# WL-Amigo/waifu2x-converter-cpp

Measured on AMD Instinct MI355X. Metric: Mpixels/sec end-to-end scale2.0x 7-layer conv, higher is better.
Workload: dtype f32; 1 GPU; scale2x_1080p (BASELINE.json configs[1]): scale2.0x topology (1-32-32-64-64-128-128-1, synthetic seeded weights) on a 1920x1080 RGB frame -> Y plane nearest-2x -> 3840x2160 CNN plane, one frame per GPU per step

## Files before the change

waifu2x-converter-cpp_amd/csrc/w2xc_wino4_body.inc:

```
    static_assert(!PROG || FUSE7, "PROG finishes the fused last layer");
    constexpr int ROWS = 16;
    constexpr int NST = CIN / 4;
    constexpr int NOB = COUT / 64;
    constexpr int CHS = 168;
    constexpr int RAW_PIECES = 11;
    constexpr unsigned RAW_BYTES = RAW_PIECES * 1024;
    constexpr unsigned U_BASE = 3 * RAW_BYTES, U_BYTES = 36 * 1024;
    constexpr unsigned V_BASE = U_BASE + 2 * U_BYTES, V_BYTES = 18 * 1024;
    constexpr unsigned SPARE_BASE = V_BASE + 2 * V_BYTES;
    constexpr unsigned BIAS_BASE = SPARE_BASE + V_BYTES;
    static_assert(CIN % 16 == 0 && COUT % 64 == 0 && NST % 4 == 0 && NST >= 8, "planes");
    constexpr int STRIP = 16;
    constexpr int GW = 8;
    constexpr unsigned TRIG_BASE = BIAS_BASE + COUT * 4;
    const int tiles_y = W4B_SEL(bd.items, nitems) / (NOB * tiles_x);
    W4B_ONLY(const int img_tiles = bd.items / NOB;)
    const int pxcd = blockIdx.x & 7;
    auto band_lo = [&](int k, int r) { return (k * tiles_x + (r & 7)) >> 3; };
    auto tile_coords = [&](int pt_, int &ty_, int &tx_) {
        W4B_ONLY(pt_ = pt_ % img_tiles;)
        if constexpr (PROG) {
            const int p8 = pt_ / tiles_x;
            int rem = pt_ - p8 * tiles_x, j = 0, lo = band_lo(pxcd, 0), wd = band_lo(pxcd + 1, 0) - lo;
            while (rem >= wd && j < 7) {
                rem -= wd;
                j++;
                lo = band_lo(pxcd, j);
                wd = band_lo(pxcd + 1, j) - lo;
            }
            ty_ = 8 * p8 + j;
            tx_ = lo + rem;
            return;
        }
        const int per_strip = STRIP * tiles_y;
        int sidx = pt_ / per_strip;
        const int nfull = tiles_x / STRIP;
        if (sidx > nfull) sidx = nfull;
        const int wid = sidx < nfull ? STRIP : tiles_x - nfull * STRIP;
        const int q = pt_ - sidx * per_strip;
        ty_ = q / wid;
        tx_ = sidx * STRIP + (q - ty_ * wid);
    };
    extern __shared__ __attribute__((aligned(16))) float lds[];
    const unsigned lds0 = (unsigned)(size_t)(__attribute__((address_space(3))) float *)lds;
    char *ldsb = reinterpret_cast<char *>(lds);

    const int lane = threadIdx.x & 63;
    const int wave = __builtin_amdgcn_readfirstlane(threadIdx.x >> 6);
    const int pt = wave & 3, bt = wave >> 2;
    const unsigned b_voff = (unsigned)lane * 16u;
    auto lin = [&]() { unsigned v = b_voff; asm volatile("" : "+v"(v)); return v; };
    auto lane_o = [&]() { return (int)(lin() >> 4); };

    const int xcd = blockIdx.x & 7, per = gridDim.x >> 3;
    const int cq = nitems >> 3, cr = nitems & 7;
    int chunk_begin = xcd < cr ? xcd * (cq + 1) : cr * (cq + 1) + (xcd - cr) * cq;
    int chunk_end = chunk_begin + cq + (xcd < cr ? 1 : 0);
    if constexpr (PROG) {
        int nloc = (tiles_y >> 3) * tiles_x;
        for (int j = 0; j < (tiles_y & 7); j++) nloc += band_lo(xcd + 1, j) - band_lo(xcd, j);
        chunk_begin = 0;
        chunk_end = nloc * NOB;
    }
#ifndef W4_PAIR
#define W4_PAIR 0
#endif
    int item0 = chunk_begin + (blockIdx.x >> 3);
    int nmy = (chunk_end - item0 + per - 1) / per;
    if constexpr (W4_PAIR && NOB == 2 && !PROG) {
        const int ntile = nitems >> 1, tq = ntile >> 3, tr = ntile & 7;
        const int tb = xcd < tr ? xcd * (tq + 1) : tr * (tq + 1) + (xcd - tr) * tq, te = tb + tq + (xcd < tr ? 1 : 0);
        item0 = tb + (blockIdx.x >> 3);
        if (item0 >= te) return;
        nmy = 2 * ((te - item0 + per - 1) / per);
    } else if (item0 >= chunk_end) return;
    auto item_of = [&](int n) {
        const int nn = n < nmy ? n : nmy - 1;
        if constexpr (W4_PAIR && NOB == 2 && !PROG) return 2 * (item0 + (nn >> 1) * per) + (nn & 1);
        else return item0 + nn * per;
    };

    for (int c = threadIdx.x; c < COUT; c += 512) lds[BIAS_BASE / 4 + c] = d.bias[c];
    if constexpr (PROG) {
        if (threadIdx.x < 4) lds[TRIG_BASE / 4 + threadIdx.x] = 0.0f;
    }

    const long long cs4 = d.in_cs * 4, rs4 = d.in_rs * 4;
    constexpr int DW = W4_DMA4 ? 4 : 8;
    constexpr int RJ = (RAW_PIECES + DW - 1) / DW;
    constexpr int UQ = 36 / DW + (36 % DW ? 1 : 0);
    unsigned voff[RJ];
    const char *a_base;
    int xlim_r;
    auto tile_offsets = [&](int it) {
        int ty_, tx_;
        tile_coords(it / NOB, ty_, tx_);
        const int lane_t = lane_o();
        const int y0 = ty_ * ROWS - d.wino_py + d.off_y, x0 = tx_ * 32 + d.off_x;
        const int yb = clampi(y0, 0, d.in_h - 1);
        a_base = reinterpret_cast<const char *>(d.in) + (long long)yb * rs4;
        W4B_ONLY(a_base += (long long)(it / bd.items) * bd.in_bs * 4;)
        xlim_r = d.in_w - x0;
        if constexpr (IN_NHWC) {
            xlim_r = 64;
#pragma unroll
            for (int jj = 0; jj < RJ; jj++) {
                int ci = (jj * DW + wave) * 64 + lane_t;
                ci = ci < (ROWS + 2) * 36 ? ci : (ROWS + 2) * 36 - 1;
                const int R = ci / 36, slot = ci - R * 36;
                const int x = 4 * (slot % 9) + slot / 9;
                const int gy = clampi(y0 + R, 0, d.in_h - 1) - yb;
                const int gx = clampi(x0 + x, 0, d.in_w - 1);
                voff[jj] = (unsigned)((long long)gy * rs4 + (long long)gx * (CIN * 4));
            }
            return;
        }
        const int xq_last = (d.in_w - 1) & ~3;
#pragma unroll
        for (int jj = 0; jj < RJ; jj++) {
            const int ci = (jj * DW + wave) * 64 + lane_t;
            int kk = ci / CHS;
            kk = kk < 4 ? kk : 3;
            const int rem = ci - kk * CHS;
            int R = rem / 9;
            const int q = rem - R * 9;
            R = R < ROWS + 2 ? R : ROWS + 1;
            const int gy = clampi(y0 + R, 0, d.in_h - 1) - yb;
            int gx = x0 + 4 * q;
            gx = gx < xq_last ? gx : xq_last;
            voff[jj] = (unsigned)((long long)kk * cs4 + (long long)gy * rs4 + (long long)gx * 4);
        }
    };
    const unsigned wbase = (unsigned)__builtin_amdgcn_readfirstlane(lds0 + (unsigned)wave * 1024u);
    auto dma_raw = [&](auto JJ, unsigned roff, int slice) {
        constexpr int jj = decltype(JJ)::value;
        const char *sbase = a_base + (long long)slice * (IN_NHWC ? 16 : 4 * cs4);
        lds_dma16_si<jj * DW * 1024u>(sbase, voff[jj], wbase + roff);
    };
    const char *wpk_w = reinterpret_cast<const char *>(d.wpk) + (size_t)wave * 1024;
    auto dma_u = [&](int ob, int s_, auto SLOT, auto Q) {
        constexpr unsigned slot = decltype(SLOT)::value;
        constexpr int q = decltype(Q)::value;
        const char *sbase = wpk_w + ((size_t)(ob * NST + s_) * 36 + q * DW) * 1024;
        lds_dma16_si<U_BASE + slot * U_BYTES + q * DW * 1024u>(sbase, b_voff, wbase);
    };
#ifndef W4_DMA_BASES
#define W4_DMA_BASES 1
#endif
    constexpr bool DMAB = W4_DMA_BASES && W4_DMA4 && !(CIN == 32 && COUT == 128 && !OUT_PLANAR && !IN_NHWC && !FUSE7);
    auto dma_u_pair = [&](const char *u_pair, auto SLOT, auto Q) {
        constexpr unsigned slot = decltype(SLOT)::value;
        constexpr int q = decltype(Q)::value;
        lds_dma16_sio<U_BASE + slot * U_BYTES + q * DW * 1024u, (q & 1) ? 0 : -(DW * 1024)>(u_pair, b_voff, wbase);
    };

    const unsigned ua_u = U_BASE + (unsigned)pt * 1024u, va_u = V_BASE + (unsigned)bt * 1024u;
#ifndef W4_KEEP_BASES
#define W4_KEEP_BASES 1
#endif
    unsigned ua0_v = b_voff + ua_u, ua1_v = b_voff + ua_u + U_BYTES, va_v = b_voff + va_u;
    asm volatile("" : "+v"(ua0_v), "+v"(ua1_v), "+v"(va_v));
    auto ua_of = [&](unsigned slot) { return W4_KEEP_BASES ? ldsb + (slot ? ua1_v : ua0_v) : ldsb + (lin() + (ua_u + slot * U_BYTES)); };
    auto va_of = [&](unsigned slot) { return W4_KEEP_BASES ? ldsb + va_v + slot * V_BYTES : ldsb + (lin() + (va_u + slot * V_BYTES)); };
#ifndef W4_KEEP_TR
#define W4_KEEP_TR 1
#endif
    auto tr_rd_calc = [&]() {
        const int l = lane_o(), tr_r = l >> 5, tr_k = (l >> 3) & 3, tr_c = l & 7;
        return IN_NHWC ? (unsigned)((4 * (2 * bt + tr_r) * 36 + tr_c) * 16 + tr_k * 4)
                       : (unsigned)((tr_k * CHS + 4 * (2 * bt + tr_r) * 9 + tr_c) * 16);
    };
    auto tr_wr_calc = [&]() {
        const int l = lane_o(), tr_r = l >> 5, tr_k = (l >> 3) & 3, tr_c = l & 7;
        return V_BASE + (unsigned)bt * 1024u + (unsigned)((tr_k * 16 + tr_r * 8 + tr_c) * 16);
    };
    unsigned tr_rd_v = tr_rd_calc(), tr_wr_v = tr_wr_calc();
    asm volatile("" : "+v"(tr_rd_v), "+v"(tr_wr_v));
    auto tr_rd = [&]() { return W4_KEEP_TR ? tr_rd_v : tr_rd_calc(); };
    auto tr_wr = [&]() { return W4_KEEP_TR ? tr_wr_v : tr_wr_calc(); };

    const int ngroups = (tiles_x + GW - 1) / GW;
    auto job_of_lane = [&](int item, int l, int &jr, int &jg) {
        int r, tx;
        tile_coords(item / NOB, r, tx);
        jr = r - (l & 1);
        jg = tx / GW - (l >> 1);
        return l < 4 && jr >= 0 && ((l >> 1) == 0 || ((tx & (GW - 1)) == 0 && tx > 0));
    };
    auto job_target = [&](int jr, int jg) {
        const int rows = jr + 1 < tiles_y ? 2 : 1;
        const int c1 = (jg + 1) * GW + 1;
        return NOB * rows * ((c1 < tiles_x ? c1 : tiles_x) - jg * GW);
    };
    const int njobs = tiles_y * ngroups;
    unsigned *const q_slots = d.prog_cnt + njobs, *const q_head = d.prog_cnt + 2 * njobs, *const q_tail = q_head + 1;
    unsigned *const lds_action = reinterpret_cast<unsigned *>(ldsb + TRIG_BASE), *const lds_ticket = lds_action + 1;
    constexpr int CW = 7;
    auto prog_early = [&](int item, unsigned &tick, unsigned &q0, unsigned &q1) {
        tick = 0xFFFFFFFFu;
        if (item >= 0) {
            int jr, jg;
            if (job_of_lane(item, lane_o(), jr, jg)) tick = __hip_atomic_fetch_add(d.prog_cnt + (jr * ngroups + jg), 1u, __ATOMIC_RELAXED, __HIP_MEMORY_SCOPE_AGENT);
        }
        const unsigned t = *lds_ticket;
        q0 = __hip_atomic_load(t ? q_slots + (t - 1) : q_head, __ATOMIC_RELAXED, __HIP_MEMORY_SCOPE_AGENT);
        q1 = __hip_atomic_load(q_tail, __ATOMIC_RELAXED, __HIP_MEMORY_SCOPE_AGENT);
    };
    auto prog_late = [&](int item, unsigned tick, unsigned q0, unsigned q1) {
        if (item >= 0) {
            int jr, jg;
            const bool valid = job_of_lane(item, lane_o(), jr, jg);
            if (valid && tick == (unsigned)(job_target(jr, jg) - 1)) {
                const unsigned slot = __hip_atomic_fetch_add(q_tail, 1u, __ATOMIC_RELAXED, __HIP_MEMORY_SCOPE_AGENT);
                __hip_atomic_store(q_slots + slot, (unsigned)(jr * ngroups + jg) + 1u, __ATOMIC_RELAXED, __HIP_MEMORY_SCOPE_AGENT);
            }
        }
        unsigned t = *lds_ticket, action = 0;
        if (t) {
            if (q0) { action = q0; t = 0; }
        } else if ((int)(q1 - q0) > 0) {
            unsigned h = 0;
            if (lane_o() == 0) h = __hip_atomic_fetch_add(q_head, 1u, __ATOMIC_RELAXED, __HIP_MEMORY_SCOPE_AGENT);
            h = (unsigned)__builtin_amdgcn_readfirstlane((int)h);
            t = h < (unsigned)njobs ? h + 1 : 0;
        }
        if (lane_o() == 0) { *lds_action = action; *lds_ticket = t; }
    };
    auto prog_run = [&]() {
        const unsigned action = (unsigned)__builtin_amdgcn_readfirstlane((int)*lds_action);
        if (action) {
            W4ProgJob a;
            a.G = d.out; a.ts = d.out_ts; a.gs = d.out_gs; a.rs = d.out_rs;
            a.out = d.g_out; a.out_rs = d.g_out_rs; a.bias = d.g_bias; a.flags = d.prog_flags; a.epoch = d.prog_epoch;
            a.g_h = d.g_h; a.g_w = d.g_w; a.g_off = d.g_off; a.wino_py = d.wino_py; a.ngroups = ngroups;
            w4_prog_job<NOB>(a, (int)(action - 1) / ngroups, (int)(action - 1) % ngroups);
        }
        return action;
    };

    float dd[36];
    auto raw_read = [&](const char *src, auto I_) {
        constexpr int i = decltype(I_)::value;
        if constexpr ((W4_ABL & 2) != 0) {
            static_for<0, 6>([&](auto JJ) { dd[i * 6 + decltype(JJ)::value] = (float)(i + decltype(JJ)::value); });
        } else if constexpr (IN_NHWC) {
            static_for<0, 6>([&](auto JJ) {
                constexpr int j = decltype(JJ)::value;
                dd[i * 6 + j] = *reinterpret_cast<const float *>(src + (i * 36 + (j & 3) * 9 + (j >> 2)) * 16);
            });
        } else {
            const f32x4 a = *reinterpret_cast<const f32x4 *>(src + i * 144);
            const f32x2 b = *reinterpret_cast<const f32x2 *>(src + i * 144 + 16);
            dd[i * 6 + 0] = a[0]; dd[i * 6 + 1] = a[1]; dd[i * 6 + 2] = a[2]; dd[i * 6 + 3] = a[3];
            dd[i * 6 + 4] = b[0]; dd[i * 6 + 5] = b[1];
        }
    };
    auto raw_mask = [&](int xlim) {
        if (xlim < 34) {
            const int lim = xlim - 4 * (lane_o() & 7);
            static_for<0, 36>([&](auto E) {
                constexpr int e = decltype(E)::value;
                dd[e] = (e % 6) < lim ? dd[e] : 0.0f;
            });
        }
    };
    auto row_pass = [&](auto I_) {
        constexpr int i = decltype(I_)::value;
        if constexpr (!(W4_ABL & 3)) bt6(dd[i * 6 + 0], dd[i * 6 + 1], dd[i * 6 + 2], dd[i * 6 + 3], dd[i * 6 + 4], dd[i * 6 + 5]);
        if constexpr (!(W4_ABL & 3)) asm volatile("" : "+v"(dd[i * 6 + 0]), "+v"(dd[i * 6 + 1]), "+v"(dd[i * 6 + 2]), "+v"(dd[i * 6 + 3]), "+v"(dd[i * 6 + 4]), "+v"(dd[i * 6 + 5]));
    };
    auto col_pass = [&](auto J_) {
        constexpr int j = decltype(J_)::value;
        if constexpr (!(W4_ABL & 3)) bt6(dd[0 * 6 + j], dd[1 * 6 + j], dd[2 * 6 + j], dd[3 * 6 + j], dd[4 * 6 + j], dd[5 * 6 + j]);
        if constexpr (!(W4_ABL & 3)) asm volatile("" : "+v"(dd[0 * 6 + j]), "+v"(dd[1 * 6 + j]), "+v"(dd[2 * 6 + j]), "+v"(dd[3 * 6 + j]), "+v"(dd[4 * 6 + j]), "+v"(dd[5 * 6 + j]));
    };
    auto v_write = [&](char *dst, auto Q_) {
        constexpr int q = decltype(Q_)::value;
        if constexpr (!(W4_ABL & 2))
        {
#ifdef W4_VW32
            static_for<0, 4>([&](auto E_) { constexpr int e = decltype(E_)::value; *reinterpret_cast<float *>(dst + q * 2048 + e * 4) = dd[w4p_dd_of(4 * q + e)]; });
#else
            *reinterpret_cast<f32x4 *>(dst + q * 2048) = f32x4{dd[w4p_dd_of(4 * q)], dd[w4p_dd_of(4 * q + 1)], dd[w4p_dd_of(4 * q + 2)], dd[w4p_dd_of(4 * q + 3)]};
#endif
        }
    };

    auto run = [&](auto PH_) {
    constexpr int PH = decltype(PH_)::value;
    using C0 = std::integral_constant<int, 0>;
    using C1 = std::integral_constant<int, 1>;
    using U0 = std::integral_constant<unsigned, 0u>;
    const unsigned park_u = (bt * 3 + PH - 1) < 4 ? U_BASE + U_BYTES + (unsigned)(bt * 3 + PH - 1) * 9216u : SPARE_BASE + (unsigned)(bt * 3 + PH - 1 - 4) * 9216u;
    auto park = [&]() {
        char *pa = ldsb + (lin() + park_u);
        static_for<0, 9>([&](auto Q_) {
            constexpr int q = decltype(Q_)::value;
            *reinterpret_cast<f32x4 *>(pa + q * 1024) = f32x4{dd[4 * q], dd[4 * q + 1], dd[4 * q + 2], dd[4 * q + 3]};
        });
    };
    auto unpark = [&]() {
        const char *pa = ldsb + (lin() + park_u);
        static_for<0, 9>([&](auto Q_) {
            constexpr int q = decltype(Q_)::value;
            const f32x4 v = *reinterpret_cast<const f32x4 *>(pa + q * 1024);
            dd[4 * q] = v[0]; dd[4 * q + 1] = v[1]; dd[4 * q + 2] = v[2]; dd[4 * q + 3] = v[3];
        });
    };
    auto quarter = [&](auto Q_, const char *src, char *dst, int xlim) {
        constexpr int q = decltype(Q_)::value;
        if constexpr (q == 0) {
            static_for<0, 6>([&](auto I) { raw_read(src, I); });
            raw_mask(xlim);
        }
        if constexpr (q < 2) static_for<3 * q, 3 * q + 3>([&](auto I) { row_pass(I); });
        else static_for<3 * (q - 2), 3 * (q - 2) + 3>([&](auto J) { col_pass(J); });
        if constexpr (q == 3) static_for<0, 9>([&](auto Q) { v_write(dst, Q); });
    };
    tile_offsets(item_of(0));
    int xlim_cur = xlim_r;
    auto raw_all = [&](unsigned roff, int slice) {
        if (wave < DW) {
            static_for<0, RJ - 1>([&](auto JJ) { dma_raw(JJ, roff, slice); });
            if (wave < RAW_PIECES - (RJ - 1) * DW) dma_raw(std::integral_constant<int, RJ - 1>{}, roff, slice);
        }
    };
    for (int sl = 0; sl < 3; sl++) raw_all((unsigned)sl * RAW_BYTES, sl);
    if (wave < DW) {
        const int ob0 = item_of(0) % NOB;
        static_for<0, UQ - 1>([&](auto Q) { dma_u(ob0, 0, U0{}, Q); });
        if (wave < 36 - (UQ - 1) * DW) dma_u(ob0, 0, U0{}, std::integral_constant<int, UQ - 1>{});
    }
    W2XC_WAIT_VMCNT(0);
    __builtin_amdgcn_s_barrier();
    asm volatile("" ::: "memory");
    if constexpr (PH < 3) {
        const char *src = ldsb + PH * RAW_BYTES + tr_rd();
        static_for<0, 4 - PH>([&](auto Q) { quarter(Q, src, ldsb + tr_wr(), xlim_cur); });
    }
    asm volatile("s_waitcnt lgkmcnt(0)" ::: "memory");
    __builtin_amdgcn_s_barrier();
    asm volatile("" ::: "memory");
    for (int sl = 3; sl < 6; sl++) raw_all((unsigned)(sl - 3) * RAW_BYTES, sl);
    W2XC_WAIT_VMCNT(0);
    __builtin_amdgcn_s_barrier();
    asm volatile("" ::: "memory");
    if constexpr (PH == 3) quarter(C0{}, ldsb + tr_rd(), nullptr, xlim_cur);
    asm volatile("s_waitcnt lgkmcnt(0)" ::: "memory");
    __builtin_amdgcn_s_barrier();
    asm volatile("" ::: "memory");

    constexpr int PF = W4_PF;
    static_assert(PF == 1 || PF == 2, "operand look-ahead");
    f32x4 a4[PF + 1], b4[PF + 1];
    auto load_first = [&](unsigned slot) {
        const char *ua = ua_of(slot);
        const char *va = va_of(slot);
        static_for<0, PF>([&](auto G) {
            constexpr int g = decltype(G)::value;
            const int b = PF == 2 ? g : (int)slot;
            a4[b] = *reinterpret_cast<const f32x4 *>(ua + g * 4096);
            b4[b] = *reinterpret_cast<const f32x4 *>(va + g * 2048);
        });
    };
    unsigned rd = RAW_BYTES, mid = 2 * RAW_BYTES, fr = 0;
    int stamp = 0;
    (void)stamp;
    W4_STAMP(stamp++);
    for (int n = 0; n < nmy; n++) {
        const int item = item_of(n), item_n = item_of(n + 1);
        f32x4 acc[36];

        auto stage = [&](auto J_, auto FIRST_, int s) {
            constexpr int J = decltype(J_)::value;
            constexpr bool FIRST = decltype(FIRST_)::value;
            constexpr int QT = (J - PH) & 3;
            constexpr unsigned par = J & 1, nxt = par ^ 1u;
            int u_ob = item % NOB, u_s = s + 1;
            if (s == NST - 1) { u_ob = item_n % NOB; u_s = 0; }
            const char *ua = ua_of(par);
            const char *va = va_of(par);
            const char *u_st = wpk_w + (size_t)(u_ob * NST + u_s) * 36864, *u_pair = u_st;
            if constexpr (DMAB) asm volatile("" : "+s"(u_st));
            const char *srcQ = nullptr;
            char *dstQ = nullptr;
            if constexpr (QT == 0) srcQ = ldsb + (rd + tr_rd());
            if constexpr (QT == 3) dstQ = ldsb + (tr_wr() + nxt * V_BYTES);
            const int xlimQ = s + 4 < NST ? xlim_cur : xlim_r;
            if constexpr (J == 2) {
                if (s == NST - 6) tile_offsets(item_n);
            }
            const int r_slice = s + 6 < NST ? s + 6 : s + 6 - NST;
            static_for<0, 36>([&](auto XI) {
                constexpr int xi = decltype(XI)::value;
                constexpr int g = xi >> 2;
                if constexpr (xi == 32) {
                    W4_STAMP(stamp++);
                    if constexpr ((W4_ABL & 32) != 0) W2XC_WAIT_VMCNT(0);
                    else if (wave < RAW_PIECES - (RJ - 1) * DW) wait_vmcnt_n(RJ);
                    else if (wave < DW) wait_vmcnt_n(RJ - 1);
                    asm volatile("s_waitcnt lgkmcnt(0)" ::: "memory");
                    W4_STAMP(stamp++);
                    __builtin_amdgcn_s_barrier();
                    asm volatile("" ::: "memory");
                    { const unsigned tr = rd; rd = mid; mid = fr; fr = tr; }
                    if (s != NST - 1) {
                        if constexpr (PF == 2) load_first(nxt);
                        else {
                            a4[nxt] = *reinterpret_cast<const f32x4 *>(ua_of(nxt));
                            b4[nxt] = *reinterpret_cast<const f32x4 *>(va_of(nxt));
                        }
                    }
                    W4_STAMP(stamp++);
                    __builtin_amdgcn_sched_barrier(0);
                }
                if constexpr ((xi & 3) == 0 && g + PF < 9 && !(W4_ABL & 128)) {
                    constexpr int b = PF == 2 ? (g + PF) % 3 : ((g + 1 + (int)par) & 1);
                    a4[b] = *reinterpret_cast<const f32x4 *>(ua + (g + PF) * 4096);
                    b4[b] = *reinterpret_cast<const f32x4 *>(va + (g + PF) * 2048);
                    __builtin_amdgcn_sched_barrier(0);
                }
                {
                    constexpr int b = PF == 2 ? g % 3 : ((g + (int)par) & 1);
                    if constexpr (FIRST) asm volatile("v_mfma_f32_16x16x4_f32 %0, %1, %2, 0" : "=v"(acc[xi]) : "v"(a4[b][xi & 3]), "v"(b4[b][xi & 3]));
                    else asm volatile("v_mfma_f32_16x16x4_f32 %0, %1, %2, %0" : "+v"(acc[xi]) : "v"(a4[b][xi & 3]), "v"(b4[b][xi & 3]));
                }
                __builtin_amdgcn_sched_barrier(0);
                constexpr int TSTEP = W4_DMA4 ? 1 : 2, tk = xi >= 1 && (xi - 1) % TSTEP == 0 ? (xi - 1) / TSTEP : -1;
                if constexpr (tk >= 0 && tk < UQ && !(W4_ABL & 16)) {
                    constexpr int q = tk;
                    if constexpr (DMAB) {
                        if (wave < (q == UQ - 1 ? 36 - (UQ - 1) * DW : DW)) {
                            if constexpr ((q & 1) == 0) {
                                u_pair = u_st + (q + 1) * (DW * 1024);
                                asm volatile("" : "+s"(u_pair));
                            }
                            dma_u_pair(u_pair, std::integral_constant<unsigned, nxt>{}, std::integral_constant<int, q>{});
                        }
                    } else {
                        if (wave < (q == UQ - 1 ? 36 - (UQ - 1) * DW : DW)) dma_u(u_ob, u_s, std::integral_constant<unsigned, nxt>{}, std::integral_constant<int, q>{});
                    }
                    __builtin_amdgcn_sched_barrier(0);
                }
                if constexpr (tk >= UQ && tk < UQ + RJ && !(W4_ABL & 32)) {
                    constexpr int jj = tk - UQ;
                    if (wave < (jj == RJ - 1 ? RAW_PIECES - (RJ - 1) * DW : DW)) dma_raw(std::integral_constant<int, jj>{}, fr, r_slice);
                    __builtin_amdgcn_sched_barrier(0);
                }
                if constexpr (QT == 0 && xi < 2) {
                    raw_read(srcQ, std::integral_constant<int, 3 * xi>{});
                    raw_read(srcQ, std::integral_constant<int, 3 * xi + 1>{});
                    raw_read(srcQ, std::integral_constant<int, 3 * xi + 2>{});
                    __builtin_amdgcn_sched_barrier(0);
                }
                if constexpr (xi >= W4P_T0 && xi < W4P_T0 + 3) {
                    if constexpr (QT == 0 && xi == W4P_T0) raw_mask(xlimQ);
                    if constexpr (QT < 2) row_pass(std::integral_constant<int, 3 * QT + xi - W4P_T0>{});
                    else col_pass(std::integral_constant<int, 3 * (QT - 2) + xi - W4P_T0>{});
                    __builtin_amdgcn_sched_barrier(0);
                }
                if constexpr (QT == 3 && xi >= W4P_T0 + 3 && xi < W4P_T0 + 6) {
                    v_write(dstQ, std::integral_constant<int, 3 * (xi - (W4P_T0 + 3))>{});
                    v_write(dstQ, std::integral_constant<int, 3 * (xi - (W4P_T0 + 3)) + 1>{});
                    v_write(dstQ, std::integral_constant<int, 3 * (xi - (W4P_T0 + 3)) + 2>{});
                    __builtin_amdgcn_sched_barrier(0);
                }
            });
        };
        load_first(0u);
        stage(std::integral_constant<int, 0>{}, std::true_type{}, 0);
#pragma unroll 1
        for (int s = 1; s < NST; s += 4) {
            stage(std::integral_constant<int, 1>{}, std::false_type{}, s);
            stage(std::integral_constant<int, 2>{}, std::false_type{}, s + 1);
            stage(std::integral_constant<int, 3>{}, std::false_type{}, s + 2);
            if (s + 3 < NST) stage(std::integral_constant<int, 0>{}, std::false_type{}, s + 3);
        }
        asm volatile("s_nop 15\n\ts_nop 15" ::: "memory");
        xlim_cur = xlim_r;
        if constexpr (PH != 0) park();
        {
            __builtin_amdgcn_s_setprio(2);
            const int ob = item % NOB;
            const int lane_e = lane_o(), t = lane_e & 15, k = lane_e >> 4;
            int tile_y, tile_x;
            tile_coords(item / NOB, tile_y, tile_x);
            const int ty0 = tile_y * ROWS - d.wino_py;
            const int oy = ty0 + 4 * (2 * bt + (t >> 3)), ox = tile_x * 32 + 4 * (t & 7);
            const int plane0 = ob * 64 + pt * 16 + 4 * k;
            float *obase = OUT_PLANAR ? W4B_OUT + (long long)plane0 * d.out_cs + (long long)oy * d.out_rs + ox
                                      : W4B_OUT + (long long)oy * d.out_rs + (long long)ox * COUT + plane0;
            const bool interior = ty0 >= 0 && ty0 + ROWS <= d.out_h && tile_x * 32 + 32 <= d.out_w;
            const f32x4 bq = *reinterpret_cast<const f32x4 *>(ldsb + BIAS_BASE + plane0 * 4);
            float a7[4];
            if constexpr (FUSE7) {
                const float *w7 = reinterpret_cast<const float *>(d.w7pk) + (size_t)(ob * 4 + pt) * 256 + lane_e;
#pragma unroll
                for (int e = 0; e < 4; e++) a7[e] = w7[e * 64];
            }
            char *red = ldsb + V_BASE + V_BYTES;
            unsigned tick = 0xFFFFFFFFu, pq0 = 0, pq1 = 0;
            (void)tick; (void)pq0; (void)pq1;
            float tm[4][6][4];
#pragma unroll
            for (int e = 0; e < 4; e++)
#pragma unroll
                for (int j = 0; j < 6; j++) {
                    const float m0 = acc[xi_of(0, j)][e], m1 = acc[xi_of(1, j)][e], m2 = acc[xi_of(2, j)][e], m3 = acc[xi_of(3, j)][e],
                                m4 = acc[xi_of(4, j)][e], m5 = acc[xi_of(5, j)][e];
                    const float s1 = m1 + m2, d1 = m1 - m2, s2 = m3 + m4, d2 = m3 - m4;
                    tm[0][j][e] = m0 + s1 + s2;
                    tm[1][j][e] = __builtin_fmaf(1.5f, d2, 0.75f * d1);
                    tm[2][j][e] = __builtin_fmaf(2.25f, s2, 0.5625f * s1);
                    tm[3][j][e] = __builtin_fmaf(3.375f, d2, __builtin_fmaf(0.421875f, d1, m5));
                }
            if constexpr (PROG) W2XC_WAIT_VMCNT(0);
#pragma unroll
            for (int rp = 0; rp < 2; rp++) {
#pragma unroll
                for (int rr = 0; rr < 2; rr++) {
                    const int i = 2 * rp + rr;
                    f32x4 y[4];
#pragma unroll
                    for (int e = 0; e < 4; e++) {
                        float y0, y1, y2, y3;
                        at6(tm[i][0][e], tm[i][1][e], tm[i][2][e], tm[i][3][e], tm[i][4][e], tm[i][5][e], y0, y1, y2, y3);
                        const float w0 = y0 + bq[e], w1 = y1 + bq[e], w2 = y2 + bq[e], w3 = y3 + bq[e];
                        const float l0 = __builtin_amdgcn_fmed3f(w0, 0.1f * w0, 3.402823466e+38f), l1 = __builtin_amdgcn_fmed3f(w1, 0.1f * w1, 3.402823466e+38f);
                        const float l2 = __builtin_amdgcn_fmed3f(w2, 0.1f * w2, 3.402823466e+38f), l3 = __builtin_amdgcn_fmed3f(w3, 0.1f * w3, 3.402823466e+38f);
                        if constexpr (OUT_PLANAR || FUSE7) y[e] = f32x4{l0, l1, l2, l3};
                        else { y[0][e] = l0; y[1][e] = l1; y[2][e] = l2; y[3][e] = l3; }
                    }
                    if constexpr (FUSE7) {
                        f32x4 D[4];
#pragma unroll
                        for (int j = 0; j < 4; j++) D[j] = f32x4{0.0f, 0.0f, 0.0f, 0.0f};
#pragma unroll
                        for (int e = 0; e < 4; e++)
#pragma unroll
                            for (int j = 0; j < 4; j++) D[j] = __builtin_amdgcn_mfma_f32_16x16x4f32(a7[e], y[e][j], D[j], 0, 0, 0);
                        const int p0 = (2 * bt + (t >> 3)) * 32 + (t & 7) * 4;
                        if (k < 2) {
#pragma unroll
                            for (int r = 0; r < 4; r++) *reinterpret_cast<f32x4 *>(red + ((pt * 9 + 4 * k + r) * 128 + p0) * 4) = f32x4{D[0][r], D[1][r], D[2][r], D[3][r]};
                        } else if (k == 2) {
                            *reinterpret_cast<f32x4 *>(red + ((pt * 9 + 8) * 128 + p0) * 4) = f32x4{D[0][0], D[1][0], D[2][0], D[3][0]};
                        }
                        asm volatile("s_waitcnt lgkmcnt(0)" ::: "memory");
                        __builtin_amdgcn_s_barrier();
                        asm volatile("" ::: "memory");
                        if constexpr (PROG) {
                            if (i == 0 && wave == CW) prog_early(n > 0 ? item_of(n - 1) : -1, tick, pq0, pq1);
                            if (i == 3 && wave == CW) prog_late(n > 0 ? item_of(n - 1) : -1, tick, pq0, pq1);
                        }
                        {
                            const int tid = wave * 64 + lane_e;
                            if (tid < 288) {
                                const int tap = tid >> 5, p = (tid & 31) * 4;
                                const int gy = ty0 + 4 * (p >> 5) + i, gx = tile_x * 32 + (p & 31);
                                f32x4 sum = *reinterpret_cast<const f32x4 *>(red + ((0 * 9 + tap) * 128 + p) * 4);
#pragma unroll
                                for (int q = 1; q < 4; q++) sum += *reinterpret_cast<const f32x4 *>(red + ((q * 9 + tap) * 128 + p) * 4);
                                if (gy >= 0 && gy < d.out_h && gx < d.out_w) {
                                    float *g = W4B_OUT + (long long)ob * d.out_ts + (long long)tap * d.out_gs + (long long)gy * d.out_rs + gx;
                                    if constexpr (PROG) {
                                        if (gx + 3 < d.out_w) store16_sc1(g, sum);
                                        else {
#pragma unroll
                                            for (int e = 0; e < 3; e++)
                                                if (gx + e < d.out_w) store4_sc1(g + e, sum[e]);
                                        }
                                    } else if (gx + 3 < d.out_w) *reinterpret_cast<f32x4u *>(g) = sum;
                                    else {
#pragma unroll
                                        for (int e = 0; e < 3; e++)
                                            if (gx + e < d.out_w) g[e] = sum[e];
                                    }
                                }
                            }
                        }
                        asm volatile("s_waitcnt lgkmcnt(0)" ::: "memory");
                        __builtin_amdgcn_s_barrier();
                        asm volatile("" ::: "memory");
                    } else if constexpr ((W4_ABL & 64) != 0) {
                        if (y[0][0] == 12345.678f) *reinterpret_cast<f32x4 *>(obase) = y[0] + y[1] + y[2] + y[3];
                    } else if constexpr (OUT_PLANAR) {
                        if (interior || (oy + i >= 0 && oy + i < d.out_h && ox < d.out_w)) {
#pragma unroll
                            for (int e = 0; e < 4; e++) *reinterpret_cast<f32x4 *>(obase + (long long)e * d.out_cs + (long long)i * d.out_rs) = y[e];
                        }
                    } else if (interior) {
#pragma unroll
                        for (int j = 0; j < 4; j++) *reinterpret_cast<f32x4 *>(obase + (long long)i * d.out_rs + j * COUT) = y[j];
                    } else {
#pragma unroll
                        for (int j = 0; j < 4; j++)
                            if (oy + i >= 0 && oy + i < d.out_h && ox + j < d.out_w) *reinterpret_cast<f32x4 *>(obase + (long long)i * d.out_rs + j * COUT) = y[j];
                    }
                }
            }
            __builtin_amdgcn_s_setprio(0);
            W4_STAMP(stamp++);
            if constexpr (PROG) prog_run();
        }
        if constexpr (PH != 0) unpark();
        asm volatile("s_waitcnt lgkmcnt(0)" ::: "memory");
        __builtin_amdgcn_s_barrier();
        asm volatile("" ::: "memory");
    }
    W2XC_WAIT_VMCNT(0);
    if constexpr (PROG) {
        __builtin_amdgcn_s_barrier();
        asm volatile("" ::: "memory");
        bool first = true;
        for (;;) {
            if (wave == CW) {
                unsigned tick, q0, q1;
                prog_early(first ? item_of(nmy - 1) : -1, tick, q0, q1);
                prog_late(first ? item_of(nmy - 1) : -1, tick, q0, q1);
                unsigned t = *lds_ticket;
                if (*lds_action == 0 && t) {
                    unsigned q = 0;
                    while ((q = __hip_atomic_load(q_slots + (t - 1), __ATOMIC_RELAXED, __HIP_MEMORY_SCOPE_AGENT)) == 0) __builtin_amdgcn_s_sleep(8);
                    if (lane_o() == 0) { *lds_action = q; *lds_ticket = 0; }
                }
            }
            const bool was_first = first;
            first = false;
            asm volatile("s_waitcnt lgkmcnt(0)" ::: "memory");
            __builtin_amdgcn_s_barrier();
            asm volatile("" ::: "memory");
            const unsigned ran = prog_run();
            __builtin_amdgcn_s_barrier();
            asm volatile("" ::: "memory");
            if (!ran && !was_first) break;
        }
    }
    };
#ifdef W4_ONE_PH
    run(std::integral_constant<int, W4_ONE_PH>{});
    return;
#endif
    switch ((pt - 2 * bt) & 3) {
    case 0: run(std::integral_constant<int, 0>{}); break;
    case 1: run(std::integral_constant<int, 1>{}); break;
    case 2: run(std::integral_constant<int, 2>{}); break;
    default: run(std::integral_constant<int, 3>{}); break;
    }
```

Before: 150.3 Mpix/s (input-image pixels; CNN-plane pixels = 4x).

## Batch fused last-layer tap reduction per item and drop park/unpark for non-PROG

For the fused 7th-layer path without progressive scheduling, partial MFMA results from all four row iterations are written to a larger per-item LDS slab that reuses U/V buffer space. A single reduction pass then runs after one barrier, replacing the two barriers and small reduction done per row iteration. The non-PROG path also stops parking the dd registers to LDS and unparking them; it pins them in VGPRs instead and recomputes the lane base offsets after each item. This removes barriers and LDS round trips, at the cost of higher register pressure and reuse of LDS regions that must not be live at that point.

```diff
diff --git a/waifu2x-converter-cpp_amd/csrc/w2xc_wino4_body.inc b/waifu2x-converter-cpp_amd/csrc/w2xc_wino4_body.inc
--- a/waifu2x-converter-cpp_amd/csrc/w2xc_wino4_body.inc
+++ b/waifu2x-converter-cpp_amd/csrc/w2xc_wino4_body.inc
@@ -158,8 +158,7 @@
 #ifndef W4_KEEP_BASES
 #define W4_KEEP_BASES 1
 #endif
-    unsigned ua0_v = b_voff + ua_u, ua1_v = b_voff + ua_u + U_BYTES, va_v = b_voff + va_u;
-    asm volatile("" : "+v"(ua0_v), "+v"(ua1_v), "+v"(va_v));
+    unsigned ua0_v = 0, ua1_v = 0, va_v = 0;
     auto ua_of = [&](unsigned slot) { return W4_KEEP_BASES ? ldsb + (slot ? ua1_v : ua0_v) : ldsb + (lin() + (ua_u + slot * U_BYTES)); };
     auto va_of = [&](unsigned slot) { return W4_KEEP_BASES ? ldsb + va_v + slot * V_BYTES : ldsb + (lin() + (va_u + slot * V_BYTES)); };
 #ifndef W4_KEEP_TR
@@ -174,8 +173,17 @@
         const int l = lane_o(), tr_r = l >> 5, tr_k = (l >> 3) & 3, tr_c = l & 7;
         return V_BASE + (unsigned)bt * 1024u + (unsigned)((tr_k * 16 + tr_r * 8 + tr_c) * 16);
     };
-    unsigned tr_rd_v = tr_rd_calc(), tr_wr_v = tr_wr_calc();
-    asm volatile("" : "+v"(tr_rd_v), "+v"(tr_wr_v));
+    unsigned tr_rd_v = 0, tr_wr_v = 0;
+    auto lane_regs = [&]() {
+        if constexpr (W4_KEEP_BASES) {
+            ua0_v = lin() + ua_u; ua1_v = lin() + (ua_u + U_BYTES); va_v = lin() + va_u;
+            asm volatile("" : "+v"(ua0_v), "+v"(ua1_v), "+v"(va_v));
+        }
+        if constexpr (W4_KEEP_TR) {
+            tr_rd_v = tr_rd_calc(); tr_wr_v = tr_wr_calc();
+            asm volatile("" : "+v"(tr_rd_v), "+v"(tr_wr_v));
+        }
+    };
     auto tr_rd = [&]() { return W4_KEEP_TR ? tr_rd_v : tr_rd_calc(); };
     auto tr_wr = [&]() { return W4_KEEP_TR ? tr_wr_v : tr_wr_calc(); };
 
@@ -286,11 +294,23 @@
         }
     };
 
+    constexpr bool PARK = PROG;
+    auto pin_dd = [&]() {
+        float(&v)[36] = dd;
+        asm volatile("" : "+v"(v[0]), "+v"(v[1]), "+v"(v[2]), "+v"(v[3]), "+v"(v[4]), "+v"(v[5]));
+        asm volatile("" : "+v"(v[6]), "+v"(v[7]), "+v"(v[8]), "+v"(v[9]), "+v"(v[10]), "+v"(v[11]));
+        asm volatile("" : "+v"(v[12]), "+v"(v[13]), "+v"(v[14]), "+v"(v[15]), "+v"(v[16]), "+v"(v[17]));
+        asm volatile("" : "+v"(v[18]), "+v"(v[19]), "+v"(v[20]), "+v"(v[21]), "+v"(v[22]), "+v"(v[23]));
+        asm volatile("" : "+v"(v[24]), "+v"(v[25]), "+v"(v[26]), "+v"(v[27]), "+v"(v[28]), "+v"(v[29]));
+        asm volatile("" : "+v"(v[30]), "+v"(v[31]), "+v"(v[32]), "+v"(v[33]), "+v"(v[34]), "+v"(v[35]));
+    };
+
     auto run = [&](auto PH_) {
     constexpr int PH = decltype(PH_)::value;
     using C0 = std::integral_constant<int, 0>;
     using C1 = std::integral_constant<int, 1>;
     using U0 = std::integral_constant<unsigned, 0u>;
+    lane_regs();
     const unsigned park_u = (bt * 3 + PH - 1) < 4 ? U_BASE + U_BYTES + (unsigned)(bt * 3 + PH - 1) * 9216u : SPARE_BASE + (unsigned)(bt * 3 + PH - 1 - 4) * 9216u;
     auto park = [&]() {
         char *pa = ldsb + (lin() + park_u);
@@ -478,7 +498,10 @@
         }
         asm volatile("s_nop 15\n\ts_nop 15" ::: "memory");
         xlim_cur = xlim_r;
-        if constexpr (PH != 0) park();
+        if constexpr (PH != 0) {
+            if constexpr (PARK) park();
+            else pin_dd();
+        }
         {
             __builtin_amdgcn_s_setprio(2);
             const int ob = item % NOB;
@@ -498,7 +521,35 @@
 #pragma unroll
                 for (int e = 0; e < 4; e++) a7[e] = w7[e * 64];
             }
+            constexpr bool SLAB_ITEM = FUSE7 && !PARK;
+            constexpr int SLAB_PX = SLAB_ITEM ? 512 : 128;
             char *red = ldsb + V_BASE + V_BYTES;
+            auto slab_of = [&](int q) {
+                if constexpr (SLAB_ITEM) return ldsb + (q < 2 ? U_BASE + U_BYTES + (unsigned)q * V_BYTES : V_BASE + V_BYTES + (unsigned)(q - 2) * V_BYTES);
+                else return red + q * (9 * 128 * 4);
+            };
+            static_assert(SPARE_BASE == V_BASE + 2 * V_BYTES && U_BYTES == 2 * V_BYTES && V_BYTES == 9 * 512 * 4, "the item's slab");
+            auto tap_reduce = [&](int job, int tap, int gy, int gx) {
+                f32x4 sum = *reinterpret_cast<const f32x4 *>(slab_of(0) + job * 16);
+#pragma unroll
+                for (int q = 1; q < 4; q++) sum += *reinterpret_cast<const f32x4 *>(slab_of(q) + job * 16);
+                if (gy >= 0 && gy < d.out_h && gx < d.out_w) {
+                    float *g = W4B_OUT + (long long)ob * d.out_ts + (long long)tap * d.out_gs + (long long)gy * d.out_rs + gx;
+                    if constexpr (PROG) {
+                        if (gx + 3 < d.out_w) store16_sc1(g, sum);
+                        else {
+#pragma unroll
+                            for (int e = 0; e < 3; e++)
+                                if (gx + e < d.out_w) store4_sc1(g + e, sum[e]);
+                        }
+                    } else if (gx + 3 < d.out_w) *reinterpret_cast<f32x4u *>(g) = sum;
+                    else {
+#pragma unroll
+                        for (int e = 0; e < 3; e++)
+                            if (gx + e < d.out_w) g[e] = sum[e];
+                    }
+                }
+            };
             unsigned tick = 0xFFFFFFFFu, pq0 = 0, pq1 = 0;
             (void)tick; (void)pq0; (void)pq1;
             float tm[4][6][4];
@@ -539,49 +590,33 @@
                         for (int e = 0; e < 4; e++)
 #pragma unroll
                             for (int j = 0; j < 4; j++) D[j] = __builtin_amdgcn_mfma_f32_16x16x4f32(a7[e], y[e][j], D[j], 0, 0, 0);
-                        const int p0 = (2 * bt + (t >> 3)) * 32 + (t & 7) * 4;
+                        const int p0 = (SLAB_ITEM ? i * 128 : 0) + (2 * bt + (t >> 3)) * 32 + (t & 7) * 4;
+                        char *slab = slab_of(pt);
                         if (k < 2) {
 #pragma unroll
-                            for (int r = 0; r < 4; r++) *reinterpret_cast<f32x4 *>(red + ((pt * 9 + 4 * k + r) * 128 + p0) * 4) = f32x4{D[0][r], D[1][r], D[2][r], D[3][r]};
+                            for (int r = 0; r < 4; r++) *reinterpret_cast<f32x4 *>(slab + ((4 * k + r) * SLAB_PX + p0) * 4) = f32x4{D[0][r], D[1][r], D[2][r], D[3][r]};
                         } else if (k == 2) {
-                            *reinterpret_cast<f32x4 *>(red + ((pt * 9 + 8) * 128 + p0) * 4) = f32x4{D[0][0], D[1][0], D[2][0], D[3][0]};
+                            *reinterpret_cast<f32x4 *>(slab + (8 * SLAB_PX + p0) * 4) = f32x4{D[0][0], D[1][0], D[2][0], D[3][0]};
                         }
-                        asm volatile("s_waitcnt lgkmcnt(0)" ::: "memory");
-                        __builtin_amdgcn_s_barrier();
-                        asm volatile("" ::: "memory");
-                        if constexpr (PROG) {
-                            if (i == 0 && wave == CW) prog_early(n > 0 ? item_of(n - 1) : -1, tick, pq0, pq1);
-                            if (i == 3 && wave == CW) prog_late(n > 0 ? item_of(n - 1) : -1, tick, pq0, pq1);
-                        }
-                        {
-                            const int tid = wave * 64 + lane_e;
-                            if (tid < 288) {
-                                const int tap = tid >> 5, p = (tid & 31) * 4;
-                                const int gy = ty0 + 4 * (p >> 5) + i, gx = tile_x * 32 + (p & 31);
-                                f32x4 sum = *reinterpret_cast<const f32x4 *>(red + ((0 * 9 + tap) * 128 + p) * 4);
-#pragma unroll
-                                for (int q = 1; q < 4; q++) sum += *reinterpret_cast<const f32x4 *>(red + ((q * 9 + tap) * 128 + p) * 4);
-                                if (gy >= 0 && gy < d.out_h && gx < d.out_w) {
-                                    float *g = W4B_OUT + (long long)ob * d.out_ts + (long long)tap * d.out_gs + (long long)gy * d.out_rs + gx;
-                                    if constexpr (PROG) {
-                                        if (gx + 3 < d.out_w) store16_sc1(g, sum);
-                                        else {
-#pragma unroll
-                                            for (int e = 0; e < 3; e++)
-                                                if (gx + e < d.out_w) store4_sc1(g + e, sum[e]);
-                                        }
-                                    } else if (gx + 3 < d.out_w) *reinterpret_cast<f32x4u *>(g) = sum;
-                                    else {
-#pragma unroll
-                                        for (int e = 0; e < 3; e++)
-                                            if (gx + e < d.out_w) g[e] = sum[e];
-                                    }
+                        if constexpr (!SLAB_ITEM) {
+                            asm volatile("s_waitcnt lgkmcnt(0)" ::: "memory");
+                            __builtin_amdgcn_s_barrier();
+                            asm volatile("" ::: "memory");
+                            if constexpr (PROG) {
+                                if (i == 0 && wave == CW) prog_early(n > 0 ? item_of(n - 1) : -1, tick, pq0, pq1);
+                                if (i == 3 && wave == CW) prog_late(n > 0 ? item_of(n - 1) : -1, tick, pq0, pq1);
+                            }
+                            {
+                                const int tid = wave * 64 + lane_e;
+                                if (tid < 288) {
+                                    const int tap = tid >> 5, p = (tid & 31) * 4;
+                                    tap_reduce(tid, tap, ty0 + 4 * (p >> 5) + i, tile_x * 32 + (p & 31));
                                 }
                             }
+                            asm volatile("s_waitcnt lgkmcnt(0)" ::: "memory");
+                            __builtin_amdgcn_s_barrier();
+                            asm volatile("" ::: "memory");
                         }
-                        asm volatile("s_waitcnt lgkmcnt(0)" ::: "memory");
-                        __builtin_amdgcn_s_barrier();
-                        asm volatile("" ::: "memory");
                     } else if constexpr ((W4_ABL & 64) != 0) {
                         if (y[0][0] == 12345.678f) *reinterpret_cast<f32x4 *>(obase) = y[0] + y[1] + y[2] + y[3];
                     } else if constexpr (OUT_PLANAR) {
@@ -599,14 +634,36 @@
                     }
                 }
             }
+            if constexpr (SLAB_ITEM) {
+                asm volatile("s_waitcnt lgkmcnt(0)" ::: "memory");
+                __builtin_amdgcn_s_barrier();
+                asm volatile("" ::: "memory");
+                const int tid = wave * 64 + lane_e;
+#pragma unroll
+                for (int jb = 0; jb < 3; jb++) {
+                    const int job = tid + jb * 512;
+                    if (jb < 2 || job < 9 * 128) {
+                        const int tap = job >> 7, i = (job >> 5) & 3, p = (job & 31) * 4;
+                        tap_reduce(job, tap, ty0 + 4 * (p >> 5) + i, tile_x * 32 + (p & 31));
+                    }
+                }
+                asm volatile("s_waitcnt lgkmcnt(0)" ::: "memory");
+                __builtin_amdgcn_s_barrier();
+                asm volatile("" ::: "memory");
+            }
             __builtin_amdgcn_s_setprio(0);
             W4_STAMP(stamp++);
             if constexpr (PROG) prog_run();
         }
-        if constexpr (PH != 0) unpark();
-        asm volatile("s_waitcnt lgkmcnt(0)" ::: "memory");
-        __builtin_amdgcn_s_barrier();
-        asm volatile("" ::: "memory");
+        if constexpr (PARK) {
+            if constexpr (PH != 0) unpark();
+            asm volatile("s_waitcnt lgkmcnt(0)" ::: "memory");
+            __builtin_amdgcn_s_barrier();
+            asm volatile("" ::: "memory");
+        } else {
+            if constexpr (PH != 0) pin_dd();
+            lane_regs();
+        }
     }
     W2XC_WAIT_VMCNT(0);
     if constexpr (PROG) {
```

New measurement: 153.3 Mpix/s (input-image pixels; CNN-plane pixels = 4x) (median of 6 runs). 1.02x the previous value.
